# JiuTongBro/vqnerf_release

Hardware: AMD Instinct MI355X
Metric: rays/sec (render) 800x800, 64+64 samples/ray, NeuS SDF 8x256 + colour 4x256 (higher is better)
Workload: dtype f32; 1 GPU; BASELINE configs[1], nerf/hotdog-shaped NeuS render: one whole 800x800 pin-hole view per rank per step (camera at distance 4, fov 0.6911), n_samples=64, n_importance=64, up_sample_steps=4, sdf 8x256; parallelism=views x1 (no data-path collective)

## Files before the change

include/vqnerf_hip.h:

```cpp
#ifndef VQNERF_HIP_H_
#define VQNERF_HIP_H_
#include <stdint.h>
#ifdef __cplusplus
extern "C" {
#endif

int vqn_version(void);
const char* vqn_last_error(void);


int vqn_vq_assign(const float* x, int64_t N, int D, const float* codebook, int K, const float* sel_mask,
                  float* ws, int64_t* idx, float* quant, float* dist, void* stream);

int vqn_vq_assign_variant(int D, int K, int has_sel_mask, int has_dist);

int vqn_vq_ema_stats(const float* x, const int64_t* idx, int64_t N, int D, int K, float* counts, float* dw,
                     float* ws, int64_t ws_bytes, void* stream);
int64_t vqn_vq_ema_stats_ws_bytes(int64_t N, int D, int K);

#define VQN_STE_WS_FLOATS 1024
int vqn_vq_ste_loss(const float* x, const float* quant, int64_t numel, float scale, float* ste, float* loss, float* ws,
                    void* stream);

int vqn_vq_ema_update(const float* counts, const float* dw, const float* codebook, int D, int K, double decay, float eps,
// ... 98 lines not shown
                              const float* pts, const float* dirs, int64_t P, int S, void* scratch,
                              int64_t scratch_bytes, float* out_sdf, float* out_grad, float* out_rgb, void* stream);

int vqn_neus_sdf_points_x3(const int32_t* sdf_desc, const float* wbuf_sdf, const float* rays_o, const float* rays_d,
                           const float* z, const float* pts, int64_t P, int S, float* out_sdf, void* stream);
int vqn_neus_fine_points_x3(const int32_t* sdf_desc, const float* wbuf_sdf, const int32_t* col_desc,
                            const float* wbuf_col, const float* rays_o, const float* rays_d, const float* z,
                            const float* pts, const float* dirs, int64_t P, int S, void* scratch,
                            int64_t scratch_bytes, float* out_sdf, float* out_grad, float* out_rgb, void* stream);

int vqn_neus_train_fwd_x3(const int32_t* sdf_desc, const float* wbuf_sdf, const int32_t* col_desc, const float* wbuf_col,
                          const float* pts, const float* dirs, int64_t P, void* scratch, int64_t scratch_bytes,
                          float* const* tensors, int n_tensors, int e_tiles, int outf_tiles, int extr_tiles, float* out_sdf,
                          float* out_n, float* out_rgb, void* stream);


typedef struct vqn_neus_pack vqn_neus_pack;
int vqn_neus_pack_create(const int32_t* sdf_dims, int sdf_n_lin, int sdf_skip, int multires, float scale, int col_mode,
                         int col_d_hidden, int col_n_layers, int multires_view, int squeeze_out, int f16s, vqn_neus_pack** out);
int vqn_neus_pack_update(vqn_neus_pack* pack, const float* const* sdf_w, const float* const* sdf_b, const float* const* col_w,
                         const float* const* col_b, void* stream);
const int32_t* vqn_neus_pack_sdf_desc(const vqn_neus_pack* pack);
const int32_t* vqn_neus_pack_col_desc(const vqn_neus_pack* pack);
const float* vqn_neus_pack_sdf_wbuf(const vqn_neus_pack* pack);
const float* vqn_neus_pack_col_wbuf(const vqn_neus_pack* pack);
int64_t vqn_neus_pack_sdf_floats(const vqn_neus_pack* pack);
int64_t vqn_neus_pack_col_floats(const vqn_neus_pack* pack);
void vqn_neus_pack_destroy(vqn_neus_pack* pack);

int64_t vqn_neus_sdf_pack_plan(const int32_t* dims, int n_lin, int skip, int multires, float scale, int max_tiles, int with_reverse,
                               int f16s, int32_t* desc_out, int32_t* words_out, int64_t words_cap);
int64_t vqn_neus_col_pack_plan(int d_feature, int mode, int d_hidden, int n_layers, int d_out, int multires_view, int squeeze_out,
                               int feat_tiles, int f16s, int32_t* desc_out, int32_t* words_out, int64_t words_cap);

int vqn_mlp_chain_vq_fwd(const int32_t* desc_a, const float* wbuf_a, const int32_t* desc_b, const float* wbuf_b, const float* in,
                         int64_t N, float* const* outs_a, const int32_t* ld_a, float* const* outs_b, const int32_t* ld_b,
                         const float* cb_frags, int K, float eps, float loss_scale, int64_t* idx, float* ste, float* loss,
                         float* counts, float* ws, void* stream);
#define VQN_VQ_FRAGS_FLOATS(K) (((K) <= 16 ? 1 : ((K) <= 32 ? 2 : 4)) * (16 * 64 * 4 + 16))
int vqn_vq_codebook_frags(const float* codebook, int D, int K, float* frags, void* stream);

int vqn_linear2srgb(const float* x, int64_t n, float* y, void* stream);


#define VQN_CHAIN_MAX_STACKS 8
typedef struct vqn_chain_stack {
  int32_t kind, n_layers;
  int32_t widths[8], acts[8];
  int32_t skip_at, input, out_slot;
} vqn_chain_stack;
typedef struct vqn_chain_pack vqn_chain_pack;
int vqn_chain_pack_create(int in_mode, int in_feats, int n_freqs, int n_stacks, const vqn_chain_stack* stacks, vqn_chain_pack** out);
int vqn_chain_pack_update(vqn_chain_pack* pack, const float* const* kernels, const float* const* biases, void* stream);
int vqn_chain_pack_n_weights(const vqn_chain_pack* pack);
const int32_t* vqn_chain_pack_desc(const vqn_chain_pack* pack);
const float* vqn_chain_pack_wbuf(const vqn_chain_pack* pack);
int64_t vqn_chain_pack_floats(const vqn_chain_pack* pack);
void vqn_chain_pack_destroy(vqn_chain_pack* pack);
int64_t vqn_chain_pack_plan(int in_mode, int in_feats, int n_freqs, int n_stacks, const vqn_chain_stack* stacks, int32_t* desc_out,
                            int32_t* words_out, int64_t words_cap);


int vqn_neus_upsample(const float* rays_o, const float* rays_d, const float* z, const float* sdf, int64_t B, int n,
                      float r_limit, float inv_s, const float* u, int n_new, float* z_new, void* stream);

int vqn_neus_merge(const float* z, const float* sdf, const float* z_new, const float* sdf_new, int64_t B, int n,
// ... 85 lines not shown
```

vqnerf_release_amd/_C.py:

```python
import contextlib
import ctypes
import os
import re

import numpy as np
import torch

_HERE = os.path.dirname(os.path.abspath(__file__))
LIB_PATH = os.environ.get('VQN_LIB', os.path.join(_HERE, 'lib', 'libvqnerf_hip.so'))
_lib = None

_ABI = """
i vqn_version()  s vqn_last_error()  i vqn_vq_assign(plipipppppp)  i vqn_vq_assign_variant(iiii)  i vqn_vq_ema_stats(ppliippplp)
l vqn_vq_ema_stats_ws_bytes(lii)  i vqn_vq_ste_loss(pplfpppp)  i vqn_vq_ema_update(pppiidfpppppppp)
i vqn_decomp_loss_fwd(ppppppliiffffffpp)  i vqn_decomp_loss_bwd(ppppppliiffffffpppppp)  i vqn_l2_normalize_rows(plifpp)
i vqn_l2_normalize_rows_bwd(pplifpp)  i vqn_vq_ste_loss_bwd(pppplpp)  i vqn_codebook_prep(ppiifpp)  i vqn_sim_smooth_fwd(piifpp)
i vqn_sim_smooth_bwd(pppiifpp)  i vqn_vq_quantize_rows(plipipffpppppp)  i vqn_vq_train_bwd(pppppflifpp)
i vqn_vq_quantize_rows_train(plipipfffppppppp)  i vqn_mlp_chain_fwd(ppplpipipipip)  i vqn_mlp_chain_fwd_f16s(ppplpipipipip)
i vqn_brdf_shade_fwd(pppppppliippppppppppppipipp)  i vqn_brdf_shade_fwd_rows(ppppppppliippppppppppppipipp)
l vqn_brdf_shade_bwd_partials(l)  i vqn_brdf_shade_bwd(pppppppliipppppppppppppppp)  i vqn_neus_sdf_points(pppppplipp)
l vqn_neus_fine_scratch_bytes(p)  i vqn_neus_fine_points(pppppppppliplpppp)  i vqn_neus_train_fwd(pppppplplpiiiipppp)
l vqn_neus_train_bwd_scratch_bytes(p)  i vqn_neus_train_bwd(ppppppplplpipip)  l vqn_neus_train_bwd_x3_scratch_bytes(p)
i vqn_neus_train_bwd_x3(pppppppplplpipip)  i vqn_pack_x3_gather(pplpp)  i vqn_pack_x3_gather2(pplpplpp)
i vqn_neus_sdf_points_f16s(pppppplipp)  i vqn_neus_fine_points_f16s(pppppppppliplpppp)  i vqn_neus_sdf_points_x3(pppppplipp)
i vqn_neus_fine_points_x3(pppppppppliplpppp)  i vqn_neus_train_fwd_x3(pppppplplpiiiipppp)  i vqn_neus_pack_create(piiifiiiiiip)
i vqn_neus_pack_update(pppppp)  p vqn_neus_pack_sdf_desc(p)  p vqn_neus_pack_col_desc(p)  p vqn_neus_pack_sdf_wbuf(p)
p vqn_neus_pack_col_wbuf(p)  l vqn_neus_pack_sdf_floats(p)  l vqn_neus_pack_col_floats(p)  v vqn_neus_pack_destroy(p)
l vqn_neus_sdf_pack_plan(piiifiiippl)  l vqn_neus_col_pack_plan(iiiiiiiiippl)  i vqn_mlp_chain_vq_fwd(ppppplpppppiffpppppp)
i vqn_vq_codebook_frags(piipp)  i vqn_linear2srgb(plpp)  i vqn_chain_pack_create(iiiipp)  i vqn_chain_pack_update(pppp)
i vqn_chain_pack_n_weights(p)  p vqn_chain_pack_desc(p)  p vqn_chain_pack_wbuf(p)  l vqn_chain_pack_floats(p)
v vqn_chain_pack_destroy(p)  l vqn_chain_pack_plan(iiiipppl)  i vqn_neus_upsample(ppppliffpipp)  i vqn_neus_merge(ppppliippp)
i vqn_neus_section_mids(plifpppp)  i vqn_neus_composite_fwd(pppppppppliffppppppppppp)  i vqn_neus_composite_bwd(pppppppppliffpppppppppp)
i vqn_tile_program(pppppilp)  l vqn_tile_program_grid(pl)  i vqn_weight_norm_fwd(ipppppp)  i vqn_weight_norm_bwd(ipppppppp)
i vqn_tfmt_pack(plilpip)  i vqn_tfmt_pack_delta(plilpipip)  i vqn_tfmt_unpack(piliplp)  i vqn_wgrad_partials(piiipiiilippp)
i vqn_wgrad_partials_x3(piiipiiilippp)  i vqn_wgrad_partials_batched(ipppppppplippip)  i vqn_reduce_partials(piiiplip)
i vqn_wgrad_finalize(ipppppppppppppp)  i vqn_clip_preserve(plffpp)  i vqn_loss_total(plppiiipp)  i vqn_ks_split_fwd(ppilppp)
i vqn_ks_split_bwd(ppilppppp)  i vqn_wgrad_thin_batched(ippppppppplippp)  i vqn_multi_copy(ipppp)  i vqn_refl_train_desc_ints()
i vqn_refl_train_fwd_x3(ppppplpippiip)  i vqn_refl_train_fwd_x3_zx(pppppplpipppiip)  l vqn_refl_train_bwd_x3_scratch_bytes(p)
i vqn_refl_train_bwd_x3(ppplpppipipippiiiplp)  i vqn_adam_step(ippppppppdddddiip)
"""
ABI = {name: (ret, args) for ret, name, args in re.findall(r'(\w) (\w+)\((\w*)\)', _ABI)}
_CTYPES = dict(p=ctypes.c_void_p, i=ctypes.c_int, l=ctypes.c_int64, f=ctypes.c_float, d=ctypes.c_double, s=ctypes.c_char_p, v=None)


class VqnError(RuntimeError):
    pass


def build(verbose=False):
    import subprocess
    cmd = ['make', '-C', os.path.join(_HERE, 'csrc'), '-j8']
    if not verbose:
        cmd.append('-s')
    subprocess.check_call(cmd)


def lib():
    global _lib
    if _lib is None:
        if not os.path.exists(LIB_PATH):
            raise VqnError(f'{LIB_PATH} is missing: run `python -c "import __graft_entry__ as g; g.build()"` '
                           '(or `make -C vqnerf_release_amd/csrc`). There is no non-HIP fallback.')
        L = ctypes.CDLL(LIB_PATH)
        for name, (ret, args) in ABI.items():
            f = getattr(L, name)
            f.restype, f.argtypes = _CTYPES[ret], [_CTYPES[a] for a in args]
        _lib = L
    return _lib


def require_device(t, what):
    if not t.is_cuda:
        raise VqnError(f'{what}: got a {t.device} tensor; the no-graph path runs on MI355X HIP kernels only '
                       '(there is no CPU fallback)')
    lib()


def _check(rc, name, count=False):
    if (rc > 0) if count else (rc == 0):
        return rc
    raise VqnError(f'{name} failed (rc={rc or -3}): {lib().vqn_last_error().decode()}')


def _call(name, *args, clock=True, count=False):
    with _clock(name if clock is True else clock) if clock else contextlib.nullcontext():
        rc = getattr(lib(), name)(*args, _stream())
    return _check(rc, name, count)


def _ptr(t):
    return t if t is None or isinstance(t, int) else t.data_ptr()


def _ptrs(ts, n=1):
    return (ctypes.c_void_p * max(n, len(ts)))(*[_ptr(t) for t in ts])


# ... 274 lines not shown
    if pts is not None:
        _f32c(pts, 'pts'); P, S = pts.shape[0], 1
        dev = pts.device
    else:
        _f32c(rays_o, 'rays_o'); _f32c(rays_d, 'rays_d'); _f32c(z, 'z')
        B, S = z.shape
        P = B * S
        dev = z.device
    out = torch.empty((P,), dtype=torch.float32, device=dev)
    entry = {'f32': 'vqn_neus_sdf_points', 'f16s': 'vqn_neus_sdf_points_f16s', 'x3': 'vqn_neus_sdf_points_x3'}[mode]
    _call(entry, dp, wp, _ptr(rays_o), _ptr(rays_d), _ptr(z), _ptr(pts), P, S, _ptr(out))
    return out


def neus_fine_points(sdf_desc, wbuf_sdf, col_desc, wbuf_col, rays_o=None, rays_d=None, z=None, pts=None, dirs=None, mode='f32'):
    _f32c(wbuf_sdf, 'wbuf_sdf'); _f32c(wbuf_col, 'wbuf_col')
    sdp, cdp = _host(sdf_desc), _host(col_desc)
    if pts is not None:
        _f32c(pts, 'pts'); _f32c(dirs, 'dirs'); P, S = pts.shape[0], 1
        dev = pts.device
    else:
        _f32c(rays_o, 'rays_o'); _f32c(rays_d, 'rays_d'); _f32c(z, 'z')
        B, S = z.shape
        P = B * S
        dev = z.device
    buf = _scratch('fine', _scratch_bytes('vqn_neus_fine_scratch_bytes', sdp), dev)
    sdf = torch.empty((P,), dtype=torch.float32, device=dev)
    grad = torch.empty((P, 3), dtype=torch.float32, device=dev)
    rgb = torch.empty((P, 3), dtype=torch.float32, device=dev)
    entry = {'f32': 'vqn_neus_fine_points', 'f16s': 'vqn_neus_fine_points_f16s', 'x3': 'vqn_neus_fine_points_x3'}[mode]
    _call(entry, sdp, _ptr(wbuf_sdf), cdp, _ptr(wbuf_col), _ptr(rays_o), _ptr(rays_d), _ptr(z), _ptr(pts), _ptr(dirs), P, S, _ptr(buf),
          buf.numel(), _ptr(sdf), _ptr(grad), _ptr(rgb))
    return sdf, grad, rgb


class NeusPackHandle:

    def __init__(self, sdf_dims, sdf_skip, multires, scale, col_mode, col_d_hidden, col_n_layers, multires_view, squeeze_out, engine):
        L = lib()
        self.h = ctypes.c_void_p()
        _check(L.vqn_neus_pack_create(_host(sdf_dims), len(sdf_dims) - 1, sdf_skip, multires, scale, col_mode, col_d_hidden, col_n_layers,
                                      multires_view, int(squeeze_out), engine, ctypes.byref(self.h)), 'vqn_neus_pack_create')
        self.sdf_desc, self.col_desc = L.vqn_neus_pack_sdf_desc(self.h), L.vqn_neus_pack_col_desc(self.h)
        self.sdf_wbuf, self.col_wbuf = L.vqn_neus_pack_sdf_wbuf(self.h), L.vqn_neus_pack_col_wbuf(self.h)

    def update(self, W, b, Wc, bc):
        for t in W + b + Wc + bc:
            _f32c(t, 'weight / bias')
        _call('vqn_neus_pack_update', self.h, _ptrs(W), _ptrs(b), _ptrs(Wc), _ptrs(bc))

    def __del__(self):
        try:
            if self.h:
                lib().vqn_neus_pack_destroy(self.h)
        except Exception:
            pass


def neus_train_fwd(sdf_desc, wbuf_sdf, col_desc, wbuf_col, pts, dirs, saved, e_tiles, outf_tiles, extr_tiles, out_sdf, out_n, out_rgb, pack=None):
    _f32c(pts, 'pts'); _f32c(dirs, 'dirs')
    for t in saved + [out_sdf, out_n, out_rgb]:
        _f32c(t, 'saved tensor')
    if pack is not None:
        sdp, cdp, wsp, wcp, entry = pack.sdf_desc, pack.col_desc, pack.sdf_wbuf, pack.col_wbuf, 'vqn_neus_train_fwd_x3'
    else:
        _f32c(wbuf_sdf, 'wbuf_sdf'); _f32c(wbuf_col, 'wbuf_col')
# ... 367 lines not shown
```

vqnerf_release_amd/csrc/neus_mlp.hip:

```cpp
#include "mlp_prims.h"
#include "vqn_neus_desc.h"
#include <stdlib.h>

using namespace eng;

#ifdef VQN_STAMPS
__device__ unsigned long long g_stamps[8];
#define VQN_STAMP_DECL unsigned long long st_[6] = {0, 0, 0, 0, 0, 0}; unsigned long long st_prev = __builtin_amdgcn_s_memtime(); const unsigned long long st_begin = st_prev;
#define VQN_STAMP(i) { const unsigned long long st_now = __builtin_amdgcn_s_memtime(); st_[i] += st_now - st_prev; st_prev = st_now; }
#define VQN_STAMP_FLUSH if (threadIdx.x == 0) { st_[5] = __builtin_amdgcn_s_memtime() - st_begin; for (int i_ = 0; i_ < 6; ++i_) atomicAdd(&g_stamps[i_], st_[i_]); atomicAdd(&g_stamps[6], 1ull); }
extern "C" int vqn_debug_read_stamps(unsigned long long* out, int reset) {
  if (hipMemcpyFromSymbol(out, HIP_SYMBOL(g_stamps), sizeof(unsigned long long) * 8) != hipSuccess) return -3;
  if (reset) { unsigned long long z[8] = {0, 0, 0, 0, 0, 0, 0, 0}; if (hipMemcpyToSymbol(HIP_SYMBOL(g_stamps), z, sizeof(z)) != hipSuccess) return -3; }
  return 0;
}
#else
#define VQN_STAMP_DECL
#define VQN_STAMP(i)
#define VQN_STAMP_FLUSH
#endif

#ifdef VQN_STAMPS
__device__ unsigned long long g_stamps2[16];
#define FS_DECL unsigned long long fs_[16] = {0, 0, 0, 0, 0, 0, 0, 0, 0, 0, 0, 0, 0, 0, 0, 0}; unsigned long long fs_prev = __builtin_amdgcn_s_memtime(); const unsigned long long fs_begin = fs_prev;
// ... 312 lines not shown
        }
    }
#pragma unroll
    for (int rq = 0; rq < 4; ++rq) {
      lds[(tmp_row0 + wave * 4 + rq) * 64 + lane] = acc_quad(acc0, rq);
      lds[IS + (tmp_row0 + wave * 4 + rq) * 64 + lane] = acc_quad(acc1, rq);
    }
  }
  __syncthreads();
  for (int r = wave; r < 8 * emb_tiles; r += 8) {
    const int im = r / (4 * emb_tiles), er = r - im * 4 * emb_tiles, tt = er >> 2, rq = er & 3;
    f32x4* li = lds + (size_t)im * IS;
    f32x4 sum = li[(tmp_row0 + tt * 4 + rq) * 64 + lane];
    for (int k = 1; k < KS; ++k) sum += li[(tmp_row0 + (k * emb_tiles + tt) * 4 + rq) * 64 + lane];
    if (accumulate) sum += li[(e_row0 + er) * 64 + lane];
    li[(e_row0 + er) * 64 + lane] = sum;
  }
  __syncthreads();
}

struct TrainOut {
  float* E; float* OUTF; float* EXTR;
  float* U[VQN_MAX_SDF_LAYERS]; float* GH[VQN_MAX_SDF_LAYERS]; float* C[VQN_MAX_COL_LAYERS];
  int e_tiles, outf_tiles, extr_tiles;
};

__device__ __forceinline__ void tfmt_store_quad(float* __restrict__ T, const long ptile, const int n_ft, const int ft, const int rq,
                                                const int lane, const f32x4 v) {
  float* base = T + ((ptile * n_ft + ft) * 32 + 8 * rq) * 32 + lane;
#pragma unroll
  for (int j = 0; j < 4; ++j) __builtin_nontemporal_store(v[j], base + 64 * j);
}

template <bool FINE, bool TRAIN = false>
__global__ __launch_bounds__(512, 1) void neus_points2_kernel(
    const SdfDesc sd, const ColDesc cd, const f32x4* __restrict__ wsdf, const f32x4* __restrict__ wcol,
    const float* __restrict__ rays_o, const float* __restrict__ rays_d, const float* __restrict__ zv,
    const float* __restrict__ pts_direct, const float* __restrict__ dirs_direct, const long P, const int S,
    f32x4* __restrict__ scratch, float* __restrict__ out_sdf, float* __restrict__ out_grad,
    float* __restrict__ out_rgb, const TrainOut to) {
  extern __shared__ __attribute__((aligned(16))) f32x4 lds[];
  const int MT = sd.max_tiles;
  const int IMG = E_ROWS + 8 * MT, IS = IMG * 64;
  const int X0 = E_ROWS, Y0 = E_ROWS + 4 * MT;
  Smalls2* sm = reinterpret_cast<Smalls2*>(lds + (size_t)2 * IS);
  const int tid = threadIdx.x, lane = tid & 63, h = lane >> 5, p = lane & 31;
  const int wave = __builtin_amdgcn_readfirstlane(tid >> 6);
  const int img = wave >> 2, w4 = wave & 3;
  f32x4* ldsi = lds + (size_t)img * IS;
  const int n_lin = sd.n_lin;
  const int emb_tiles = (sd.emb_feats + 31) >> 5;
  const long n_tiles = (P + 31) >> 5, n_pairs = (n_tiles + 1) >> 1;
  const size_t per_img = (size_t)(n_lin - 1) * 4 * MT * 64;
#ifdef VQN_DIAG_STASH_ROT
  f32x4* save0 = nullptr;
#else
  f32x4* save0 = FINE ? scratch + (size_t)blockIdx.x * 2 * per_img : nullptr;
#endif
  const int feat_slot = (n_lin - 2) * 4 * MT;
  f32x4 pre[4];
  f32x4 nopre[4];

  FS_DECL
  for (long pair = blockIdx.x; pair < n_pairs; pair += gridDim.x) {
#ifdef VQN_DIAG_STASH_ROT
    if (FINE) save0 = scratch + ((size_t)((pair / gridDim.x) % VQN_DIAG_STASH_ROT) * gridDim.x + blockIdx.x) * 2 * per_img;
#endif
    FS(12)
    if (tid < 64) {
      const int im = tid >> 5, t = tid & 31;
      long pt = ((2 * pair + im) << 5) + t;
      if (pt >= P) pt = P - 1;
      float x, y, z, dx = 0.f, dy = 0.f, dz = 0.f;
      if (pts_direct != nullptr) {
        x = pts_direct[pt * 3 + 0]; y = pts_direct[pt * 3 + 1]; z = pts_direct[pt * 3 + 2];
        if (FINE) { dx = dirs_direct[pt * 3 + 0]; dy = dirs_direct[pt * 3 + 1]; dz = dirs_direct[pt * 3 + 2]; }
      } else {
        const long ray = pt / S;
        const float tt = zv[pt];
        dx = rays_d[ray * 3 + 0]; dy = rays_d[ray * 3 + 1]; dz = rays_d[ray * 3 + 2];
        x = rays_o[ray * 3 + 0] + __fmul_rn(dx, tt);
        y = rays_o[ray * 3 + 1] + __fmul_rn(dy, tt);
        z = rays_o[ray * 3 + 2] + __fmul_rn(dz, tt);
      }
      sm->pts[im][t * 3 + 0] = x; sm->pts[im][t * 3 + 1] = y; sm->pts[im][t * 3 + 2] = z;
      sm->dirs[im][t * 3 + 0] = dx; sm->dirs[im][t * 3 + 1] = dy; sm->dirs[im][t * 3 + 2] = dz;
    }
    __syncthreads();
    const float xs = sm->pts[img][p * 3 + 0] * sd.scale, ys = sm->pts[img][p * 3 + 1] * sd.scale, zs = sm->pts[img][p * 3 + 2] * sd.scale;
    const long ptile_w = 2 * pair + img;
    for (int r = w4; r < (TRAIN ? 4 * to.e_tiles : sd.emb_rows); r += 4) {
      f32x4 v;
// ... 18 lines not shown
      const LayerDesc L = sd.layers[l];
      const f32x4* next_wp = nullptr;
      if (l + 1 < n_lin - 1 && wave < sd.layers[l + 1].n_out_tiles)
        next_wp = wsdf + sd.layers[l + 1].w_off + (size_t)wave * (4 * L.n_out_tiles + ((l + 1 == sd.skip) ? sd.emb_rows : 0)) * 64 + lane;
      const KSegs ks = (l == 0) ? KSegs{E0, sd.emb_rows, 0, 0}
                                : KSegs{cur, 4 * sd.layers[l - 1].n_out_tiles, E0, (l == sd.skip) ? sd.emb_rows : 0};
      const int dst = (l == 0) ? X0 : oth;
      const bool do_save = FINE && (l < n_lin - 2);
      const f32x4* bp = wsdf + L.b_off;
      float* const t_u = TRAIN ? to.U[l + 1] : nullptr;
      auto bias_init = [&](int ot, int im, f32x16& acc) { if (im == 0) { FS(2) } init_bias(bp, ot, lane, acc); };
      auto epi_rq = [&](int ot, int im, int rq, const f32x16& acc) {
        if (im == 0 && rq == 0) { FS(1) }
        f32x4* li = lds + (size_t)im * IS;
        f32x4* sv = save0 + (size_t)im * per_img + (size_t)l * 4 * MT * 64;
        f32x4 v = {acc[4 * rq], acc[4 * rq + 1], acc[4 * rq + 2], acc[4 * rq + 3]};
#pragma unroll
        for (int j = 0; j < 4; ++j) v[j] = act_fwd<ACT_SOFTPLUS100>(v[j]);
        li[(dst + ot * 4 + rq) * 64 + lane] = v;
        if (do_save) st_stream(sv + (ot * 4 + rq) * 64 + lane, v);
        if (TRAIN && 2 * pair + im < n_tiles) tfmt_store_quad(t_u, 2 * pair + im, L.n_out_tiles, ot, rq, lane, v);
      };
      gemm_tiles2<8>(lds, IS, ks, wsdf + L.w_off, L.n_out_tiles, wave, lane, pre, true, next_wp, bias_init, epi_rq);
      FS(2)
      __syncthreads();
      FS(3)
      if (l == 0) { cur = X0; oth = Y0; } else { const int t = cur; cur = oth; oth = t; }
    }
    const int hid_rows = 4 * sd.layers[n_lin - 2].n_out_tiles;

    rowdot<1>(ldsi, cur, hid_rows, wsdf + sd.last_w_off, sm->part[img], w4, lane);
    if (FINE && sd.layers[n_lin - 1].n_out_tiles > 0) {
      const LayerDesc L = sd.layers[n_lin - 1];
      const f32x4* bp = wsdf + L.b_off;
      gemm_tiles2<8>(lds, IS, KSegs{cur, hid_rows, 0, 0}, wsdf + L.w_off, L.n_out_tiles, wave, lane, nopre, false, nullptr,
                     [&](int ot, int, f32x16& acc) { init_bias(bp, ot, lane, acc); },
                     [&](int ot, int im, int rq, const f32x16& acc) {
                       f32x4* sv = save0 + (size_t)im * per_img + (size_t)feat_slot * 64;
                       const f32x4 v = {acc[4 * rq], acc[4 * rq + 1], acc[4 * rq + 2], acc[4 * rq + 3]};
                       st_stream(sv + (ot * 4 + rq) * 64 + lane, v);
                       if (TRAIN && 2 * pair + im < n_tiles) {
                         float* base = to.OUTF + (2 * pair + im) * (long)to.outf_tiles * 1024;
#pragma unroll
                         for (int j = 0; j < 4; ++j) {
                           const int f = 32 * ot + 2 * (4 * rq + j) + h + 1;
                           if (f < 32 * to.outf_tiles) __builtin_nontemporal_store(v[j], base + f * 32 + p);
                         }
                       }
                     });
    }
    __syncthreads();
    if (tid < 64) {
      const int im = tid >> 5, t = tid & 31;
      const long pt = ((2 * pair + im) << 5) + t;
      if (pt < P) {
        const float* pr = sm->part[im];
        const float s = ((pr[t] + pr[32 + t]) + (pr[64 + t] + pr[96 + t])) + (sd.last_b_off > 0 ? wsdf[sd.last_b_off][0] : sd.last_bias);
        out_sdf[pt] = s / sd.scale;
      }
      if (TRAIN && 2 * pair + im < n_tiles) {
        float* base = to.OUTF + (2 * pair + im) * (long)to.outf_tiles * 1024;
        const float* pr = sm->part[im];
        base[t] = ((pr[t] + pr[32 + t]) + (pr[64 + t] + pr[96 + t])) + (sd.last_b_off > 0 ? wsdf[sd.last_b_off][0] : sd.last_bias);
        for (int f = 32 * sd.layers[n_lin - 1].n_out_tiles + 1; f < 32 * to.outf_tiles; ++f) base[f * 32 + t] = 0.f;
      }
    }
    if (!FINE) { __syncthreads(); FS(4) continue; }
    FS(4)
// ... 65 lines not shown
      for (int k = 0; k < sd.multires; ++k) {
        const int fs = 3 + 6 * k + c, fc = fs + 3;
        g = fmaf(G(fs), posenc_jac(fs, x0, x1, x2, &cc), g);
        g = fmaf(G(fc), posenc_jac(fc, x0, x1, x2, &cc), g);
      }
      sm->grad[im][pp * 3 + c] = g;
      const long pt = ((2 * pair + im) << 5) + pp;
      if (pt < P) out_grad[pt * 3 + c] = g;
    }
    __syncthreads();
    FS(9)
    if (cd.n_lin == 0) continue;

    {
      const float px = sm->pts[img][p * 3 + 0], py = sm->pts[img][p * 3 + 1], pz = sm->pts[img][p * 3 + 2];
      const float dx = sm->dirs[img][p * 3 + 0], dy = sm->dirs[img][p * 3 + 1], dz = sm->dirs[img][p * 3 + 2];
      for (int r = w4; r < (TRAIN ? 4 * to.extr_tiles : cd.extra_rows); r += 4) {
        f32x4 v;
#pragma unroll
        for (int j = 0; j < 4; ++j) {
          const int f = row_feat(r, h, j);
          float val = 0.f;
          if (r >= cd.extra_rows) val = 0.f;
          else if (f < 3) val = f == 0 ? px : (f == 1 ? py : pz);
          else if (f < 3 + cd.n_view_feats) val = posenc_feat(f - 3, dx, dy, dz);
          else if (f < cd.extra_feats) val = sm->grad[img][p * 3 + (f - 3 - cd.n_view_feats)];
          v[j] = val;
        }
        if (r < cd.extra_rows) ldsi[(E0 + r) * 64 + lane] = v;
        if (TRAIN && ptile_w < n_tiles) tfmt_store_quad(to.EXTR, ptile_w, to.extr_tiles, r >> 2, r & 3, lane, v);
      }
      const f32x4* sv = save0 + (size_t)img * per_img + (size_t)feat_slot * 64;
      const int feat_rows = 4 * sd.layers[n_lin - 1].n_out_tiles;
      for (int r0 = w4; r0 < feat_rows; r0 += 32) {
        f32x4 v[8];
#pragma unroll
        for (int c = 0; c < 8; ++c) v[c] = ld_stream(sv + min(r0 + 4 * c, feat_rows - 1) * 64 + lane);
#pragma unroll
        for (int c = 0; c < 8; ++c)
          if (r0 + 4 * c < feat_rows) ldsi[(X0 + r0 + 4 * c) * 64 + lane] = v[c];
      }
      __syncthreads();
      FS(10)
      cur = X0; oth = Y0;
      int in_rows = feat_rows;
      for (int l = 0; l < cd.n_lin - 1; ++l) {
        const LayerDesc L = cd.layers[l];
        const KSegs ks{cur, in_rows, E0, l == 0 ? cd.extra_rows : 0};
        const f32x4* bp = wcol + L.b_off;
        const int dst = oth;
        float* const t_c = TRAIN ? to.C[l + 1] : nullptr;
        gemm_tiles2<8>(lds, IS, ks, wcol + L.w_off, L.n_out_tiles, wave, lane, nopre, false, nullptr,
                       [&](int ot, int, f32x16& acc) { init_bias(bp, ot, lane, acc); },
                       [&](int ot, int im, int rq, const f32x16& acc) {
                         f32x4* li = lds + (size_t)im * IS;
                         f32x4 v = {acc[4 * rq], acc[4 * rq + 1], acc[4 * rq + 2], acc[4 * rq + 3]};
#pragma unroll
                         for (int j = 0; j < 4; ++j) v[j] = act_fwd<ACT_RELU>(v[j]);
                         li[(dst + ot * 4 + rq) * 64 + lane] = v;
                         if (TRAIN && 2 * pair + im < n_tiles) tfmt_store_quad(t_c, 2 * pair + im, L.n_out_tiles, ot, rq, lane, v);
                       });
        __syncthreads();
        const int t = cur; cur = oth; oth = t;
        in_rows = 4 * L.n_out_tiles;
      }
      FS(11)
      rowdot<3>(ldsi, cur, in_rows, wcol + cd.last_w_off, sm->part[img], w4, lane);
      __syncthreads();
      if (tid < 192) {
        const int im = tid / 96, r = tid - 96 * im, pp = r & 31, o = r >> 5;
        const float* pr = sm->part[im];
        float v = ((pr[(0 * 32 + pp) * 3 + o] + pr[(1 * 32 + pp) * 3 + o]) + (pr[(2 * 32 + pp) * 3 + o] + pr[(3 * 32 + pp) * 3 + o])) +
                  (cd.last_b_off > 0 ? wcol[cd.last_b_off][o] : cd.last_bias[o]);
        if (cd.squeeze_out) v = 1.f / (1.f + expf(-v));
        const long pt = ((2 * pair + im) << 5) + pp;
        if (pt < P) out_rgb[pt * 3 + o] = v;
      }
    }
    __syncthreads();
// ... 108 lines not shown
  const int emb_rows = sd.emb_rows;
  if (emb_rows >= 1 && emb_rows <= 12) sd.emb_rows = 1;
  if (check_sdf_desc(sd) != 0) return -2;
#ifdef VQN_DIAG_STASH_ROT
  return (int64_t)VQN_DIAG_STASH_ROT * vqn_num_cus() * 2 * (int64_t)(sd.n_lin - 1) * 4 * sd.max_tiles * 1024;
#else
  return (int64_t)vqn_num_cus() * 2 * (int64_t)(sd.n_lin - 1) * 4 * sd.max_tiles * 1024;
#endif
}

extern "C" int vqn_neus_fine_points(const int32_t* sdf_desc, const float* wbuf_sdf, const int32_t* col_desc,
                                    const float* wbuf_col, const float* rays_o, const float* rays_d, const float* z,
                                    const float* pts, const float* dirs, int64_t P, int S, void* scratch,
                                    int64_t scratch_bytes, float* out_sdf, float* out_grad, float* out_rgb,
                                    void* stream) {
  VQN_CHECK_ARG(sdf_desc && wbuf_sdf && col_desc && wbuf_col, "descriptors and weight packs must be non-null");
  VQN_CHECK_ARG(out_sdf && out_grad && scratch, "out_sdf, out_grad and scratch must be non-null");
  VQN_CHECK_ARG(P >= 0, "P >= 0");
  if (P == 0) return VQN_OK;
  VQN_CHECK_ARG((pts != nullptr && dirs != nullptr) || (rays_o && rays_d && z && S > 0),
                "either (pts, dirs) or (rays_o, rays_d, z, S) required");
  SdfDesc sd;
  ColDesc cd;
  memcpy(&sd, sdf_desc, sizeof(SdfDesc));
  memcpy(&cd, col_desc, sizeof(ColDesc));
  VQN_CHECK_SHAPE(check_sdf_desc(sd) == 0, "invalid SDF network descriptor");
  if (cd.n_lin != 0) {
    VQN_CHECK_ARG(out_rgb != nullptr, "out_rgb must be non-null when a colour net is given");
    VQN_CHECK_SHAPE(sd.layers[sd.n_lin - 1].n_out_tiles >= 1, "SDF network has no feature outputs (d_out == 1)");
    VQN_CHECK_SHAPE(cd.n_lin >= 2 && cd.n_lin <= VQN_MAX_COL_LAYERS && cd.d_out == 3, "colour net: 2..8 layers, d_out == 3");
    VQN_CHECK_SHAPE(cd.extra_feats >= 3 && cd.extra_feats <= 64 && cd.extra_rows >= 1 && cd.extra_rows <= 8, "colour net extras");
    for (int l = 0; l < cd.n_lin - 1; ++l)
      VQN_CHECK_SHAPE(cd.layers[l].n_out_tiles >= 1 && cd.layers[l].n_out_tiles <= sd.max_tiles, "colour layer wider than max_tiles");
  }
  const long n_tiles = (P + 31) / 32;
  const int64_t per_wg = (int64_t)(sd.n_lin - 1) * 4 * sd.max_tiles * 1024;
  if (use_two_images(sd.max_tiles)) {
    const size_t lds2 = lds_bytes2(sd.max_tiles);
    VQN_HIP(hipFuncSetAttribute((const void*)neus_points2_kernel<true>, hipFuncAttributeMaxDynamicSharedMemorySize, (int)lds2));
    long grid = (long)vqn_num_cus();
    if (grid > (n_tiles + 1) / 2) grid = (n_tiles + 1) / 2;
#ifdef VQN_DIAG_STASH_ROT
    VQN_CHECK_ARG((int64_t)VQN_DIAG_STASH_ROT * grid * 2 * per_wg <= scratch_bytes, "diag build: scratch must hold ROT regions per workgroup");
#else
    if ((int64_t)grid * 2 * per_wg > scratch_bytes) grid = (long)(scratch_bytes / (2 * per_wg));
#endif
    VQN_CHECK_ARG(grid >= 1, "scratch too small (see vqn_neus_fine_scratch_bytes)");
    hipLaunchKernelGGL(neus_points2_kernel<true>, dim3((unsigned)grid), dim3(512), lds2, (hipStream_t)stream, sd, cd,
                       reinterpret_cast<const f32x4*>(wbuf_sdf), reinterpret_cast<const f32x4*>(wbuf_col), rays_o, rays_d,
                       z, pts, dirs, (long)P, S, reinterpret_cast<f32x4*>(scratch), out_sdf, out_grad, out_rgb, TrainOut{});
    VQN_LAUNCH_CHECK();
    return VQN_OK;
  }
  const size_t lds = lds_bytes(sd.max_tiles);
  VQN_CHECK_SHAPE(lds <= 160 * 1024, "network too wide for LDS");
  if (lds > 64 * 1024)
    VQN_HIP(hipFuncSetAttribute((const void*)neus_points_kernel<true>, hipFuncAttributeMaxDynamicSharedMemorySize, (int)lds));
  long grid = (long)vqn_num_cus() * 2;
  if (grid > n_tiles) grid = n_tiles;
  if ((int64_t)grid * per_wg > scratch_bytes) grid = (long)(scratch_bytes / per_wg);
  VQN_CHECK_ARG(grid >= 1, "scratch too small (see vqn_neus_fine_scratch_bytes)");
  hipLaunchKernelGGL(neus_points_kernel<true>, dim3((unsigned)grid), dim3(256), lds, (hipStream_t)stream, sd, cd,
                     reinterpret_cast<const f32x4*>(wbuf_sdf), reinterpret_cast<const f32x4*>(wbuf_col), rays_o, rays_d,
                     z, pts, dirs, (long)P, S, reinterpret_cast<f32x4*>(scratch), out_sdf, out_grad, out_rgb);
  VQN_LAUNCH_CHECK();
  return VQN_OK;
}
```

vqnerf_release_amd/geo/models/renderer.py:

```python
import warnings

import numpy as np
import torch
import torch.nn.functional as F

from vqnerf_release_amd import _C
from vqnerf_release_amd.geo import packing
from vqnerf_release_amd.geo.models.fields import _needs_graph


class CompositeFunction(torch.autograd.Function):

    @staticmethod
    def forward(ctx, sdf, grad, rgb, inv_s, rays_o, rays_d, mid_z, dists, bg, radius, car):
        sdf, grad, rgb = sdf.detach().contiguous(), grad.detach().contiguous(), rgb.detach().contiguous()
        inv_s = inv_s.detach().reshape(1).contiguous()
        o = _C.neus_composite_fwd(rays_o, rays_d, mid_z, dists, sdf, grad, rgb, inv_s, bg, radius, car)
        gsum = o['gerr'].sum(0)
        gerr = gsum[0] / (gsum[1] + 1e-5)
        ctx.save_for_backward(sdf, grad, rgb, inv_s, rays_o, rays_d, mid_z, dists, gsum[1:2].contiguous())
        ctx.bg, ctx.radius, ctx.car = bg, radius, car
        ctx.mark_non_differentiable(o['cdf'], o['inside_sphere'], o['surf'], o['depth'], o['weight_max'])
        return o['color'], o['weight_sum'], gerr, o['weights'], o['cdf'], o['inside_sphere'], o['surf'], o['depth'], o['weight_max']

    @staticmethod
    def backward(ctx, g_color, g_wsum, g_gerr, g_weights, *unused):
        sdf, grad, rgb, inv_s, rays_o, rays_d, mid_z, dists, den = ctx.saved_tensors
        B, n = mid_z.shape
        z = lambda *s: torch.zeros(s, dtype=torch.float32, device=mid_z.device)
        g_color = z(B, 3) if g_color is None else g_color.contiguous()
        gw = None if g_wsum is None else g_wsum.reshape(B).contiguous()
        gwt = None if g_weights is None else g_weights.contiguous()
# ... 35 lines not shown
    cdf = torch.cumsum(pdf, -1)
    cdf = torch.cat([torch.zeros_like(cdf[..., :1]), cdf], -1)
    if u is None:
        if det:
            u = torch.linspace(0.5 / n_samples, 1.0 - 0.5 / n_samples, steps=n_samples, device=bins.device)
            u = u.expand(list(cdf.shape[:-1]) + [n_samples])
        else:
            u = torch.rand(list(cdf.shape[:-1]) + [n_samples], device=bins.device)
    u = u.contiguous()
    inds = torch.searchsorted(cdf, u, right=True)
    below = (inds - 1).clamp(min=0)
    above = inds.clamp(max=cdf.shape[-1] - 1)
    cdf_b, cdf_a = torch.gather(cdf, -1, below), torch.gather(cdf, -1, above)
    bin_b, bin_a = torch.gather(bins, -1, below), torch.gather(bins, -1, above)
    denom = cdf_a - cdf_b
    denom = torch.where(denom < 1e-5, torch.ones_like(denom), denom)
    return bin_b + (u - cdf_b) / denom * (bin_a - bin_b)


class NeuSRenderer:
    def __init__(self, nerf, sdf_network, deviation_network, color_network, n_samples, n_importance, n_outside,
                 up_sample_steps, perturb):
        self.nerf = nerf
        self.sdf_network = sdf_network
        self.deviation_network = deviation_network
        self.color_network = color_network
        self.n_samples = n_samples
        self.n_importance = n_importance
        self.n_outside = n_outside
        self.up_sample_steps = up_sample_steps
        self.perturb = perturb
        self._u = {}
        self._engines = {}
        self._step_pack = None
        self.weights_only = False
        self.matrix_mode = 'f32'
        self.train_backend = 'hip'
        self.last_train_backend = None

    def _packs(self):
        mt, mode = self.color_network.max_tiles(), self.matrix_mode
        wb_s, d_s = self.sdf_network.packs(max_tiles=mt, mode=mode)
        wb_c, d_c = self.color_network.packs(feat_tiles=self.sdf_network.plan(mode=mode).tiles[-1], mode=mode)
        return wb_s, d_s, wb_c, d_c

    def _quantiles(self, m, device):
        key = (m, str(device))
        if key not in self._u:
            self._u[key] = torch.linspace(0.5 / m, 1.0 - 0.5 / m, steps=m, device=device).contiguous()
        return self._u[key]

    def up_sample(self, rays_o, rays_d, z_vals, sdf, r_limit, n_importance, inv_s):
        B, n = z_vals.shape
        return _C.neus_upsample(rays_o.contiguous(), rays_d.contiguous(), z_vals.contiguous(),
                                sdf.reshape(B, n).contiguous(), float(r_limit), float(inv_s),
                                self._quantiles(n_importance, z_vals.device))

    def cat_z_vals(self, rays_o, rays_d, z_vals, new_z_vals, sdf, last=False):
        if last:
            z, _ = _C.neus_merge(z_vals.contiguous(), None, new_z_vals.contiguous(), None)
            return z, sdf
        new_sdf = self._sdf_at(rays_o.contiguous(), rays_d.contiguous(), new_z_vals.contiguous()).reshape(new_z_vals.shape)
        return _C.neus_merge(z_vals.contiguous(), sdf.reshape(z_vals.shape).contiguous(), new_z_vals.contiguous(), new_sdf)

    def _sdf_pack(self):
        return self.sdf_network.packs(max_tiles=self.color_network.max_tiles(), mode=self.matrix_mode)

    def _sdf_at(self, rays_o, rays_d, z):
        if self._step_pack is not None:
            return _C.neus_sdf_points(None, None, rays_o=rays_o, rays_d=rays_d, z=z, mode='x3', pack=self._step_pack)
        wb_s, d_s = self._sdf_pack()
        return _C.neus_sdf_points(d_s, wb_s, rays_o=rays_o, rays_d=rays_d, z=z, mode=self.matrix_mode)

    @torch.no_grad()
    def _importance_z(self, rays_o, rays_d, z_vals, radius):
        B = rays_o.shape[0]
# ... 12 lines not shown
        pts = rays_o[:, None, :] + rays_d[:, None, :] * mid[..., :, None]
        r = torch.linalg.norm(pts, ord=2, dim=-1, keepdim=True).clip(1.0, 1e10)
        pts = torch.cat([pts / r, 1.0 / r], dim=-1).reshape(-1, 4)
        dirs = rays_d[:, None, :].expand(B, n, 3).reshape(-1, 3)
        density, col = nerf(pts, dirs)
        alpha = 1.0 - torch.exp(-F.softplus(density.reshape(B, n)) * dists)
        weights = alpha * torch.cumprod(torch.cat([torch.ones([B, 1], device=alpha.device), 1. - alpha + 1e-7], -1), -1)[:, :-1]
        col = col.reshape(B, n, 3)
        color = (weights[:, :, None] * col).sum(dim=1)
        if background_rgb is not None:
            color = color + background_rgb * (1.0 - weights.sum(dim=-1, keepdim=True))
        return {'color': color, 'sampled_color': col, 'alpha': alpha, 'weights': weights}

    def render_core(self, rays_o, rays_d, z_vals, sample_dist, radius, sdf_network, deviation_network, color_network,
                    background_alpha=None, background_sampled_color=None, background_rgb=None,
                    cos_anneal_ratio=0.0, to_light=False):
        if background_alpha is not None:
            self.last_train_backend = 'torch'
            return self._render_core_autograd(rays_o, rays_d, z_vals, sample_dist, radius, sdf_network, deviation_network,
                                              color_network, background_rgb, cos_anneal_ratio, to_light,
                                              background_alpha=background_alpha, background_sampled_color=background_sampled_color)
        if _needs_graph(sdf_network, rays_o) or any(p.requires_grad and torch.is_grad_enabled()
                                                    for m in (deviation_network, color_network) for p in m.parameters()):
            if self.train_backend == 'hip' and rays_o.is_cuda and self._train_engine(sdf_network, color_network) is not None:
                self.last_train_backend = 'hip'
                return self._render_core_train_hip(rays_o, rays_d, z_vals, sample_dist, radius, sdf_network,
                                                   deviation_network, color_network, background_rgb, cos_anneal_ratio, to_light)
            self.last_train_backend = 'torch'
            return self._render_core_autograd(rays_o, rays_d, z_vals, sample_dist, radius, sdf_network,
                                              deviation_network, color_network, background_rgb, cos_anneal_ratio, to_light)
        B, n = z_vals.shape
        per_ray = sample_dist.reshape(-1).float().contiguous() if to_light else None
        mid_z, dists = _C.neus_section_mids(z_vals.contiguous(), 0.0 if to_light else float(sample_dist), per_ray)
        wb_s, d_s, wb_c, d_c = self._packs()
        if self.weights_only:
            no_col = np.zeros(packing.COL_DESC_INTS, np.int32)
            sdf, grad, _ = _C.neus_fine_points(d_s, wb_s, no_col, wb_s, rays_o=rays_o, rays_d=rays_d, z=mid_z, mode=self.matrix_mode)
            rgb = torch.zeros_like(grad)
        else:
            sdf, grad, rgb = _C.neus_fine_points(d_s, wb_s, d_c, wb_c, rays_o=rays_o, rays_d=rays_d, z=mid_z, mode=self.matrix_mode)
        inv_s = torch.exp(deviation_network.variance.detach().float() * 10.0).reshape(1).contiguous()
        bg = None if background_rgb is None else background_rgb.detach().float().to(z_vals.device)
        o = _C.neus_composite_fwd(rays_o, rays_d, mid_z, dists, sdf, grad, rgb, inv_s, bg, radius, cos_anneal_ratio)
        gerr = o['gerr'].sum(0)
        inv_s_c = inv_s.clip(1e-6, 1e6)
        return {
            'color': o['color'], 'sdf': sdf.reshape(-1, 1), 'dists': dists, 'gradients': grad.reshape(B, n, 3),
            's_val': (1.0 / inv_s_c).reshape(1, 1).expand(B * n, 1), 'mid_z_vals': mid_z, 'weights': o['weights'],
            'cdf': o['cdf'], 'gradient_error': gerr[0] / (gerr[1] + 1e-5), 'inside_sphere': o['inside_sphere'],
            'surf': o['surf'], 'depth': o['depth'], 'weight_sum': o['weight_sum'], 'weight_max': o['weight_max'],
            'sampled_color': rgb.reshape(B, n, 3),
        }

    def _prepare_train_step(self, rays_o):
        if self.n_outside > 0 or self.train_backend != 'hip' or not rays_o.is_cuda or not torch.is_grad_enabled():
            return None
        sn, cn, dn = self.sdf_network, self.color_network, self.deviation_network
        if not (_needs_graph(sn, rays_o) or any(p.requires_grad for m in (dn, cn) for p in m.parameters())):
            return None
        engine = self._train_engine(sn, cn)
        if engine is None:
            return None
        return engine.prepare_step([getattr(sn, 'lin%d' % l) for l in range(sn.num_layers - 1)],
                                   [getattr(cn, 'lin%d' % l) for l in range(cn.num_layers - 1)])

    def _train_engine(self, sdf_network, color_network):
        key = (id(sdf_network), id(color_network))
# ... 143 lines not shown
```

Before: 270,600 rays/s.

## Fold SDF feature layer into colour net first layer for fine-point inference

Precomputes the product of the colour network's first-layer feature weights with the SDF network's last (feature) layer, so the fine inference kernel goes straight from the last SDF hidden layer to the colour hidden layer. The kernel computes the folded pre-activation instead of the SDF feature outputs, then adds the extra inputs (points, normals, view dirs) through a separate small GEMM before the colour MLP continues. This removes one layer's GEMM and the feature read-back in the fine path. The folded pack is cached per weight pack, computed in double on device, and can be turned off through an environment variable.

```diff
diff --git a/include/vqn_neus_fold.h b/include/vqn_neus_fold.h
--- /dev/null
+++ b/include/vqn_neus_fold.h
@@ -0,0 +1,16 @@
+#ifndef VQN_NEUS_FOLD_H_
+#define VQN_NEUS_FOLD_H_
+#include <stdint.h>
+#ifdef __cplusplus
+extern "C" {
+#endif
+
+int64_t vqn_neus_fold_pack(const int32_t* sdf_desc, const int32_t* col_desc, const float* wbuf_col, int64_t col_floats,
+                           const float* sdf_w_last, const float* sdf_b_last, int sdf_hidden, int d_feature, const float* col_w0,
+                           const float* col_b0, int col_hidden, float* wbuf_out, int64_t out_floats, int32_t* col_desc_out,
+                           void* stream);
+
+#ifdef __cplusplus
+}
+#endif
+#endif
diff --git a/include/vqnerf_hip.h b/include/vqnerf_hip.h
--- a/include/vqnerf_hip.h
+++ b/include/vqnerf_hip.h
@@ -154,6 +154,7 @@
                                int f16s, int32_t* desc_out, int32_t* words_out, int64_t words_cap);
 int64_t vqn_neus_col_pack_plan(int d_feature, int mode, int d_hidden, int n_layers, int d_out, int multires_view, int squeeze_out,
                                int feat_tiles, int f16s, int32_t* desc_out, int32_t* words_out, int64_t words_cap);
+
 
 int vqn_mlp_chain_vq_fwd(const int32_t* desc_a, const float* wbuf_a, const int32_t* desc_b, const float* wbuf_b, const float* in,
                          int64_t N, float* const* outs_a, const int32_t* ld_a, float* const* outs_b, const int32_t* ld_b,
diff --git a/vqnerf_release_amd/_C.py b/vqnerf_release_amd/_C.py
--- a/vqnerf_release_amd/_C.py
+++ b/vqnerf_release_amd/_C.py
@@ -40,6 +40,7 @@
 i vqn_refl_train_bwd_x3(ppplpppipipippiiiplp)  i vqn_adam_step(ippppppppdddddiip)
 """
 ABI = {name: (ret, args) for ret, name, args in re.findall(r'(\w) (\w+)\((\w*)\)', _ABI)}
+ABI_FOLD = {'vqn_neus_fold_pack': ('l', 'ppplppiippiplpp')}
 _CTYPES = dict(p=ctypes.c_void_p, i=ctypes.c_int, l=ctypes.c_int64, f=ctypes.c_float, d=ctypes.c_double, s=ctypes.c_char_p, v=None)
 
 
@@ -62,7 +63,7 @@
             raise VqnError(f'{LIB_PATH} is missing: run `python -c "import __graft_entry__ as g; g.build()"` '
                            '(or `make -C vqnerf_release_amd/csrc`). There is no non-HIP fallback.')
         L = ctypes.CDLL(LIB_PATH)
-        for name, (ret, args) in ABI.items():
+        for name, (ret, args) in list(ABI.items()) + list(ABI_FOLD.items()):
             f = getattr(L, name)
             f.restype, f.argtypes = _CTYPES[ret], [_CTYPES[a] for a in args]
         _lib = L
@@ -403,6 +404,19 @@
     _call(entry, sdp, _ptr(wbuf_sdf), cdp, _ptr(wbuf_col), _ptr(rays_o), _ptr(rays_d), _ptr(z), _ptr(pts), _ptr(dirs), P, S, _ptr(buf),
           buf.numel(), _ptr(sdf), _ptr(grad), _ptr(rgb))
     return sdf, grad, rgb
+
+
+def neus_fold_pack(sdf_desc, col_desc, wbuf_col, sdf_w_last, sdf_b_last, col_w0, col_b0):
+    for t in (wbuf_col, sdf_w_last, sdf_b_last, col_w0, col_b0):
+        _f32c(t, 'weight / bias')
+    (F1, H), C = sdf_w_last.shape, col_w0.shape[0]
+    sdp, cdp = _host(sdf_desc), _host(col_desc)
+    desc = np.zeros(len(col_desc), np.int32)
+    args = (sdp, cdp, _ptr(wbuf_col), wbuf_col.numel(), _ptr(sdf_w_last), _ptr(sdf_b_last), H, F1 - 1, _ptr(col_w0), _ptr(col_b0), C)
+    n = _call('vqn_neus_fold_pack', *args, None, 0, None, clock=False, count=True)
+    out = torch.empty((n,), dtype=torch.float32, device=wbuf_col.device)
+    _call('vqn_neus_fold_pack', *args, _ptr(out), n, desc.ctypes.data_as(ctypes.c_void_p), count=True)
+    return out, desc
 
 
 class NeusPackHandle:
diff --git a/vqnerf_release_amd/csrc/neus_fold.hip b/vqnerf_release_amd/csrc/neus_fold.hip
--- /dev/null
+++ b/vqnerf_release_amd/csrc/neus_fold.hip
@@ -0,0 +1,103 @@
+#include "common.h"
+#include "vqn_neus_desc.h"
+#include "vqn_neus_fold.h"
+
+namespace {
+
+struct FoldShape {
+  int H, F, C, extra;
+  int hid_rows, extra_rows, n_out_tiles;
+  int64_t base, n_w, n_b, n_e;
+};
+
+__device__ __forceinline__ int phi(int i) { return 2 * (i & 3) + 8 * (i >> 3) + ((i >> 2) & 1); }
+__device__ __forceinline__ int row_feat(int r, int h, int j) { return 32 * (r >> 2) + 2 * (4 * (r & 3) + j) + h; }
+
+__global__ __launch_bounds__(256) void neus_fold_kernel(const FoldShape s, const float* __restrict__ wbuf_col,
+                                                        const float* __restrict__ w8, const float* __restrict__ b8,
+                                                        const float* __restrict__ wc0, const float* __restrict__ bc0,
+                                                        float* __restrict__ out) {
+  const int64_t i = (int64_t)blockIdx.x * blockDim.x + threadIdx.x;
+  if (i >= s.base + s.n_w + s.n_b + s.n_e) return;
+  if (i < s.base) { out[i] = wbuf_col[i]; return; }
+  const int ldc = s.extra + s.F;
+  int64_t k = i - s.base;
+  if (k < s.n_w) {
+    const int j = (int)(k & 3), lane = (int)((k >> 2) & 63);
+    const int64_t gq = k >> 8;
+    const int g = (int)(gq % s.hid_rows), ot = (int)(gq / s.hid_rows);
+    const int c = 32 * ot + phi(lane & 31), kk = row_feat(g, lane >> 5, j);
+    double acc = 0.0;
+    if (c < s.C && kk < s.H) {
+      const float* __restrict__ a = wc0 + (size_t)c * ldc + s.extra;
+      const float* __restrict__ b = w8 + s.H + kk;
+      for (int f = 0; f < s.F; ++f) acc = fma((double)a[f], (double)b[(size_t)f * s.H], acc);
+    }
+    out[i] = (float)acc;
+    return;
+  }
+  k -= s.n_w;
+  if (k < s.n_b) {
+    const int r = (int)(k & 15), h = (int)((k >> 4) & 1), ot = (int)(k >> 5);
+    const int c = 32 * ot + 2 * r + h;
+    double acc = 0.0;
+    if (c < s.C) {
+      const float* __restrict__ a = wc0 + (size_t)c * ldc + s.extra;
+      for (int f = 0; f < s.F; ++f) acc = fma((double)a[f], (double)b8[1 + f], acc);
+      acc += (double)bc0[c];
+    }
+    out[i] = (float)acc;
+    return;
+  }
+  k -= s.n_b;
+  {
+    const int j = (int)(k & 3), lane = (int)((k >> 2) & 63);
+    const int64_t gq = k >> 8;
+    const int g = (int)(gq % s.extra_rows), ot = (int)(gq / s.extra_rows);
+    const int c = 32 * ot + phi(lane & 31), f = row_feat(g, lane >> 5, j);
+    out[i] = (c < s.C && f < s.extra) ? wc0[(size_t)c * ldc + f] : 0.0f;
+  }
+}
+
+}
+
+extern "C" int64_t vqn_neus_fold_pack(const int32_t* sdf_desc, const int32_t* col_desc, const float* wbuf_col, int64_t col_floats,
+                                      const float* sdf_w_last, const float* sdf_b_last, int sdf_hidden, int d_feature,
+                                      const float* col_w0, const float* col_b0, int col_hidden, float* wbuf_out, int64_t out_floats,
+                                      int32_t* col_desc_out, void* stream) {
+  VQN_CHECK_ARG(sdf_desc && col_desc, "descriptors must be non-null");
+  SdfDesc sd;
+  ColDesc cd;
+  memcpy(&sd, sdf_desc, sizeof(SdfDesc));
+  memcpy(&cd, col_desc, sizeof(ColDesc));
+  VQN_CHECK_SHAPE(sd.n_lin >= 2 && sd.n_lin <= VQN_MAX_SDF_LAYERS && cd.n_lin >= 2 && cd.n_lin <= VQN_MAX_COL_LAYERS, "layer counts");
+  VQN_CHECK_ARG(sdf_hidden >= 1 && d_feature >= 1 && col_hidden >= 1, "widths must be positive");
+  VQN_CHECK_ARG(col_floats > 0 && (col_floats & 3) == 0, "col_floats: the colour pack's size (a whole number of float4)");
+  FoldShape s;
+  s.H = sdf_hidden; s.F = d_feature; s.C = col_hidden; s.extra = cd.extra_feats;
+  s.hid_rows = 4 * sd.layers[sd.n_lin - 2].n_out_tiles;
+  s.extra_rows = cd.extra_rows;
+  s.n_out_tiles = cd.layers[0].n_out_tiles;
+  VQN_CHECK_SHAPE(s.hid_rows == 4 * ((s.H + 31) / 32) && sd.layers[sd.n_lin - 1].n_out_tiles == (s.F + 31) / 32 &&
+                  s.n_out_tiles == (s.C + 31) / 32, "widths do not match the descriptors' tile counts");
+  VQN_CHECK_SHAPE(s.extra >= 3 && s.extra <= 64 && s.extra_rows == (((s.extra + 1) / 2) + 3) / 4, "colour-net extras (f32 packs only)");
+  VQN_CHECK_SHAPE(cd.reserved1 == 0 && cd.reserved2 == 0 && cd.reserved3 == 0, "col_desc is folded already");
+  s.base = col_floats;
+  s.n_w = (int64_t)s.n_out_tiles * s.hid_rows * 256;
+  s.n_b = (int64_t)s.n_out_tiles * 32;
+  s.n_e = (int64_t)s.n_out_tiles * s.extra_rows * 256;
+  const int64_t total = s.base + s.n_w + s.n_b + s.n_e;
+  VQN_CHECK_SHAPE(total / 4 < (int64_t)1 << 31, "pack too large for 32-bit float4 offsets");
+  if (col_desc_out != nullptr) {
+    cd.reserved1 = (int)(s.base / 4);
+    cd.reserved2 = (int)((s.base + s.n_w) / 4);
+    cd.reserved3 = (int)((s.base + s.n_w + s.n_b) / 4);
+    memcpy(col_desc_out, &cd, sizeof(ColDesc));
+  }
+  if (wbuf_out == nullptr || out_floats < total) return total;
+  VQN_CHECK_ARG(wbuf_col && sdf_w_last && sdf_b_last && col_w0 && col_b0, "weight pointers must be non-null");
+  hipLaunchKernelGGL(neus_fold_kernel, dim3((unsigned)((total + 255) / 256)), dim3(256), 0, (hipStream_t)stream, s, wbuf_col, sdf_w_last,
+                     sdf_b_last, col_w0, col_b0, wbuf_out);
+  VQN_LAUNCH_CHECK();
+  return total;
+}
diff --git a/vqnerf_release_amd/csrc/neus_mlp.hip b/vqnerf_release_amd/csrc/neus_mlp.hip
--- a/vqnerf_release_amd/csrc/neus_mlp.hip
+++ b/vqnerf_release_amd/csrc/neus_mlp.hip
@@ -368,7 +368,7 @@
   for (int j = 0; j < 4; ++j) __builtin_nontemporal_store(v[j], base + 64 * j);
 }
 
-template <bool FINE, bool TRAIN = false>
+template <bool FINE, bool TRAIN = false, bool FOLD = false>
 __global__ __launch_bounds__(512, 1) void neus_points2_kernel(
     const SdfDesc sd, const ColDesc cd, const f32x4* __restrict__ wsdf, const f32x4* __restrict__ wcol,
     const float* __restrict__ rays_o, const float* __restrict__ rays_d, const float* __restrict__ zv,
@@ -394,6 +394,8 @@
   f32x4* save0 = FINE ? scratch + (size_t)blockIdx.x * 2 * per_img : nullptr;
 #endif
   const int feat_slot = (n_lin - 2) * 4 * MT;
+  constexpr bool fold = FOLD;
+  static_assert(!FOLD || (FINE && !TRAIN), "the fold is an inference path: the backward and the weight gradients read OUTF");
   f32x4 pre[4];
   f32x4 nopre[4];
 
@@ -478,8 +480,9 @@
     rowdot<1>(ldsi, cur, hid_rows, wsdf + sd.last_w_off, sm->part[img], w4, lane);
     if (FINE && sd.layers[n_lin - 1].n_out_tiles > 0) {
       const LayerDesc L = sd.layers[n_lin - 1];
-      const f32x4* bp = wsdf + L.b_off;
-      gemm_tiles2<8>(lds, IS, KSegs{cur, hid_rows, 0, 0}, wsdf + L.w_off, L.n_out_tiles, wave, lane, nopre, false, nullptr,
+      const f32x4* bp = fold ? wcol + cd.reserved2 : wsdf + L.b_off;
+      gemm_tiles2<8>(lds, IS, KSegs{cur, hid_rows, 0, 0}, fold ? wcol + cd.reserved1 : wsdf + L.w_off,
+                     fold ? cd.layers[0].n_out_tiles : L.n_out_tiles, wave, lane, nopre, false, nullptr,
                      [&](int ot, int, f32x16& acc) { init_bias(bp, ot, lane, acc); },
                      [&](int ot, int im, int rq, const f32x16& acc) {
                        f32x4* sv = save0 + (size_t)im * per_img + (size_t)feat_slot * 64;
@@ -611,7 +614,7 @@
       }
       const f32x4* sv = save0 + (size_t)img * per_img + (size_t)feat_slot * 64;
       const int feat_rows = 4 * sd.layers[n_lin - 1].n_out_tiles;
-      for (int r0 = w4; r0 < feat_rows; r0 += 32) {
+      for (int r0 = w4; r0 < (fold ? 0 : feat_rows); r0 += 32) {
         f32x4 v[8];
 #pragma unroll
         for (int c = 0; c < 8; ++c) v[c] = ld_stream(sv + min(r0 + 4 * c, feat_rows - 1) * 64 + lane);
@@ -623,7 +626,30 @@
       FS(10)
       cur = X0; oth = Y0;
       int in_rows = feat_rows;
-      for (int l = 0; l < cd.n_lin - 1; ++l) {
+      if (fold) {
+        const LayerDesc L = cd.layers[0];
+        const int dst = oth;
+        gemm_tiles2<8>(lds, IS, KSegs{E0, cd.extra_rows, 0, 0}, wcol + cd.reserved3, L.n_out_tiles, wave, lane, nopre, false, nullptr,
+                       [&](int ot, int im, f32x16& acc) {
+                         const f32x4* pp = save0 + (size_t)im * per_img + (size_t)feat_slot * 64 + ot * 256 + lane;
+#pragma unroll
+                         for (int rq = 0; rq < 4; ++rq) {
+                           const f32x4 v = ld_stream(pp + rq * 64);
+                           acc[4 * rq + 0] = v[0]; acc[4 * rq + 1] = v[1]; acc[4 * rq + 2] = v[2]; acc[4 * rq + 3] = v[3];
+                         }
+                       },
+                       [&](int ot, int im, int rq, const f32x16& acc) {
+                         f32x4* li = lds + (size_t)im * IS;
+                         f32x4 v = {acc[4 * rq], acc[4 * rq + 1], acc[4 * rq + 2], acc[4 * rq + 3]};
+#pragma unroll
+                         for (int j = 0; j < 4; ++j) v[j] = act_fwd<ACT_RELU>(v[j]);
+                         li[(dst + ot * 4 + rq) * 64 + lane] = v;
+                       });
+        __syncthreads();
+        const int t = cur; cur = oth; oth = t;
+        in_rows = 4 * L.n_out_tiles;
+      }
+      for (int l = fold ? 1 : 0; l < cd.n_lin - 1; ++l) {
         const LayerDesc L = cd.layers[l];
         const KSegs ks{cur, in_rows, E0, l == 0 ? cd.extra_rows : 0};
         const f32x4* bp = wcol + L.b_off;
@@ -798,12 +824,16 @@
     VQN_CHECK_SHAPE(cd.extra_feats >= 3 && cd.extra_feats <= 64 && cd.extra_rows >= 1 && cd.extra_rows <= 8, "colour net extras");
     for (int l = 0; l < cd.n_lin - 1; ++l)
       VQN_CHECK_SHAPE(cd.layers[l].n_out_tiles >= 1 && cd.layers[l].n_out_tiles <= sd.max_tiles, "colour layer wider than max_tiles");
+    VQN_CHECK_ARG((cd.reserved1 > 0 && cd.reserved2 > cd.reserved1 && cd.reserved3 > cd.reserved2) ||
+                  (cd.reserved1 == 0 && cd.reserved2 == 0 && cd.reserved3 == 0), "col_desc: fold offsets (reserved1..3) inconsistent");
   }
   const long n_tiles = (P + 31) / 32;
   const int64_t per_wg = (int64_t)(sd.n_lin - 1) * 4 * sd.max_tiles * 1024;
   if (use_two_images(sd.max_tiles)) {
     const size_t lds2 = lds_bytes2(sd.max_tiles);
-    VQN_HIP(hipFuncSetAttribute((const void*)neus_points2_kernel<true>, hipFuncAttributeMaxDynamicSharedMemorySize, (int)lds2));
+    const bool fold = cd.n_lin != 0 && cd.reserved1 > 0;
+    const auto kernel = fold ? neus_points2_kernel<true, false, true> : neus_points2_kernel<true>;
+    VQN_HIP(hipFuncSetAttribute((const void*)kernel, hipFuncAttributeMaxDynamicSharedMemorySize, (int)lds2));
     long grid = (long)vqn_num_cus();
     if (grid > (n_tiles + 1) / 2) grid = (n_tiles + 1) / 2;
 #ifdef VQN_DIAG_STASH_ROT
@@ -812,7 +842,7 @@
     if ((int64_t)grid * 2 * per_wg > scratch_bytes) grid = (long)(scratch_bytes / (2 * per_wg));
 #endif
     VQN_CHECK_ARG(grid >= 1, "scratch too small (see vqn_neus_fine_scratch_bytes)");
-    hipLaunchKernelGGL(neus_points2_kernel<true>, dim3((unsigned)grid), dim3(512), lds2, (hipStream_t)stream, sd, cd,
+    hipLaunchKernelGGL(kernel, dim3((unsigned)grid), dim3(512), lds2, (hipStream_t)stream, sd, cd,
                        reinterpret_cast<const f32x4*>(wbuf_sdf), reinterpret_cast<const f32x4*>(wbuf_col), rays_o, rays_d,
                        z, pts, dirs, (long)P, S, reinterpret_cast<f32x4*>(scratch), out_sdf, out_grad, out_rgb, TrainOut{});
     VQN_LAUNCH_CHECK();
diff --git a/vqnerf_release_amd/geo/models/renderer.py b/vqnerf_release_amd/geo/models/renderer.py
--- a/vqnerf_release_amd/geo/models/renderer.py
+++ b/vqnerf_release_amd/geo/models/renderer.py
@@ -1,3 +1,4 @@
+import os
 import warnings
 
 import numpy as np
@@ -99,16 +100,27 @@
         self.perturb = perturb
         self._u = {}
         self._engines = {}
+        self._fold = None
         self._step_pack = None
         self.weights_only = False
         self.matrix_mode = 'f32'
         self.train_backend = 'hip'
         self.last_train_backend = None
 
-    def _packs(self):
+    def _packs(self, fold=False):
         mt, mode = self.color_network.max_tiles(), self.matrix_mode
         wb_s, d_s = self.sdf_network.packs(max_tiles=mt, mode=mode)
         wb_c, d_c = self.color_network.packs(feat_tiles=self.sdf_network.plan(mode=mode).tiles[-1], mode=mode)
+        if fold and mode == 'f32' and os.environ.get('VQN_NEUS_FOLD', '1') != '0':
+            f = self._fold
+            if f is None or f[0] is not wb_s or f[1] is not wb_c:
+                sl = getattr(self.sdf_network, 'lin%d' % (self.sdf_network.num_layers - 2))
+                cl = self.color_network.lin0
+                with torch.no_grad():
+                    fw, fd = _C.neus_fold_pack(d_s, d_c, wb_c, sl.effective_weight().float().contiguous(), sl.bias.float().contiguous(),
+                                               cl.effective_weight().float().contiguous(), cl.bias.float().contiguous())
+                self._fold = f = (wb_s, wb_c, fw, fd)
+            wb_c, d_c = f[2], f[3]
         return wb_s, d_s, wb_c, d_c
 
     def _quantiles(self, m, device):
@@ -187,7 +199,7 @@
         B, n = z_vals.shape
         per_ray = sample_dist.reshape(-1).float().contiguous() if to_light else None
         mid_z, dists = _C.neus_section_mids(z_vals.contiguous(), 0.0 if to_light else float(sample_dist), per_ray)
-        wb_s, d_s, wb_c, d_c = self._packs()
+        wb_s, d_s, wb_c, d_c = self._packs(fold=not self.weights_only)
         if self.weights_only:
             no_col = np.zeros(packing.COL_DESC_INTS, np.int32)
             sdf, grad, _ = _C.neus_fine_points(d_s, wb_s, no_col, wb_s, rays_o=rays_o, rays_d=rays_d, z=mid_z, mode=self.matrix_mode)
```

New measurement: 279,600 rays/s (median of 6 runs). 1.03x the previous value.
